# 1mishra/cbc

Hardware: AMD Instinct MI355X
Metric: Mbases/s encoded (bit-exact) on synthetic 150 bp SAM (higher is better)
Workload: dtype u32; 1 GPU; cfg2: synthetic 150 bp SAM, 10000000 reads per GPU vs a 248956422 bp uniform-ACGT contig, block-parallel encode; reads_rank0=10000000, blocks_rank0=2442, block_reads=4096, lds_bytes_per_block=15264, payload_bytes_rank0=20710203, parallelism=one GPU, no collective

## Files before the change

cbc_amd/csrc/cbc_encode_body.h:

```cpp
#ifndef CBC_ENCODE_BODY_H
#define CBC_ENCODE_BODY_H

#include <stdint.h>
#include <type_traits>
#include "../../include/cbc_gpu.h"
#include "cbc_plan.h"

#ifndef CBC_PRIO_CODER
#define CBC_PRIO_CODER 3
#define CBC_PRIO_MODEL 0
#endif
#define CBC_REC_PACK_AT 56u
#define CBC_AWORD     26u
#define CBC_M26       ((1u << 26) - 1u)
#define CBC_M25       ((1u << 25) - 1u)
#define CBC_RESCALE   (1u << 20)
#define CBC_NVARCTX   0xffffu
#define CBC_NOMEMO    0xffffffffu
#define CBC_BLOOM_LOG2 13u
#define CBC_ROLE_FUSED 0u
#define CBC_ROLE_MODEL 1u
#define CBC_ROLE_CODER 2u

#define CBC_LT_MATCH   0u
// ... 68 lines not shown
}

template <class W>
struct CbcWin {
    typedef typename W::V32 V32;
#ifndef CBC_WIN_SCALAR
    V32 w;
    CBC_MFN void clear() { w = W::splat(0u); }
    CBC_MFN void shift(uint32_t d)
    {
        if (d == 0u) return;
        if (d >= 256u) { clear(); return; }
        const V32 ln = W::lane();
        const V32 src = ln + (d >> 5);
        const V32 lo = W::lane_gather(w, src), hi = W::lane_gather(w, src + 1u);
        w = W::select(ln < 8u, W::funnel_shr(hi, lo, d & 31u), W::splat(0u));
    }
    CBC_MFN uint32_t first(uint32_t p, uint32_t rl)
    {
        uint32_t out = rl + 2u;
        if (p >= rl) return out;
        const V32 ln = W::lane();
        const uint32_t pw = p >> 5;
        const V32 a = W::select(ln == pw, w & (0xffffffffu << (p & 31u)), W::select(ln > pw, w, W::splat(0u)));
        const uint64_t hb = W::ballot(a != 0u);
        if (hb) {
            const uint32_t hl = W::ctz64(hb);
            const uint32_t pos = hl * 32u + W::ctz64((uint64_t)W::readlane(a, hl));
            if (pos < rl) out = pos - p;
        }
        return out;
    }
    CBC_MFN void set(uint32_t k)
    {
        if (k < 256u) w = w | W::select(W::lane() == (k >> 5), W::splat(1u << (k & 31u)), W::splat(0u));
    }
#else
    uint64_t w0, w1, w2, w3;
    CBC_MFN void clear() { w0 = w1 = w2 = w3 = 0; }
    CBC_MFN void shift(uint32_t d)
    {
        if (d == 0u) return;
        if (d >= 256u) { clear(); return; }
        uint32_t wsh = d >> 6, bsh = d & 63u;
        if (wsh == 1u) { w0 = w1; w1 = w2; w2 = w3; w3 = 0; }
        else if (wsh == 2u) { w0 = w2; w1 = w3; w2 = 0; w3 = 0; }
        else if (wsh == 3u) { w0 = w3; w1 = 0; w2 = 0; w3 = 0; }
        if (bsh) {
            uint32_t inv = 64u - bsh;
            w0 = (w0 >> bsh) | (w1 << inv);
            w1 = (w1 >> bsh) | (w2 << inv);
            w2 = (w2 >> bsh) | (w3 << inv);
            w3 = w3 >> bsh;
        }
    }
    CBC_MFN uint32_t first(uint32_t p, uint32_t rl)
    {
        uint32_t out = rl + 2u;
        if (p >= rl) return out;
        uint32_t pw = p >> 6; uint64_t pm = ~0ull << (p & 63u);
        uint64_t a0 = pw == 0u ? (w0 & pm) : 0ull;
        uint64_t a1 = pw == 1u ? (w1 & pm) : (pw < 1u ? w1 : 0ull);
        uint64_t a2 = pw == 2u ? (w2 & pm) : (pw < 2u ? w2 : 0ull);
        uint64_t a3 = pw == 3u ? (w3 & pm) : w3;
        uint32_t pos = 0xffffffffu;
        if (a0) pos = W::ctz64(a0);
        else if (a1) pos = 64u + W::ctz64(a1);
        else if (a2) pos = 128u + W::ctz64(a2);
        else if (a3) pos = 192u + W::ctz64(a3);
        if (pos < rl) out = pos - p;
        return out;
    }
    CBC_MFN void set(uint32_t k)
    {
        uint64_t bit = 1ull << (k & 63u); uint32_t kw = k >> 6;
        w0 |= (kw == 0u) ? bit : 0ull;
        w1 |= (kw == 1u) ? bit : 0ull;
        w2 |= (kw == 2u) ? bit : 0ull;
        w3 |= (kw == 3u) ? bit : 0ull;
    }
#endif
};

template <class W, bool GEN = false>
struct CbcEnc {
    typedef typename W::V32 V32;
    typedef typename W::Mask Mask;

    typedef typename W::Uv Uv;
    Uv l, rng;
    Uv lm1;
    Uv thr0;
    CBC_MFN void set_l_forms()
    {
        lm1 = W::uv_opaque(l - 1u);
        thr0 = ((l & (1u << 24)) | (1u << 25)) - l;
    }
    uint32_t scale3;
    uint32_t bitpos, flushed;
    uint32_t *ring;
    uint32_t *out32; uint32_t cap_words;
    uint32_t status, nsym, fail_read, cur_read;
    V32 q_lo, q_cnt, q_n; uint32_t q_len;
    uint32_t role, batch_i; uint32_t *batch, *ctl;
    V32 b_lo, b_hi, b_n, b_fl, b_fh; uint32_t b_len, b_pos, b_stop, b_flags, seen_last; uint64_t b_neq;
    V32 rec_a, rec_s; uint32_t rec_n;
#ifdef CBC_STAMP
    unsigned long long t_last, t_sum[16];
#endif

    V32 small;
    V32 fkey, fexc; uint32_t fcount;
    V32 hkey, hexc; uint32_t hc0, hc1, hc2, hc3, hn0, hn1, hn2, hn3;
    uint32_t *rlen_exc, *snps_exc, *indels_exc, *rname_key, *rname_exc, *pos_val, *pos_occ, *pos_pre, *pos_idx, *var_ev, *bloom, *p0ev;
    uint32_t *runs;
    uint32_t snps_n, indels_n;
    uint32_t rn_count, rn_cap;
    uint32_t *vtab;
    uint32_t *fsp_key, *fsp_exc; uint32_t fsp_count;
    uint32_t *pos_ov_val, *pos_ov_occ; uint32_t pos_lds_cap;
    uint32_t *palpha; uint32_t pa_n0, pa_n1, pa_n2, pa_n3;
    uint32_t pos_card, cap_pos;
    uint32_t nev, nev1, cap_var;
    V32 p0cnt; uint32_t p0over;
    uint32_t L0;

    uint32_t prevPos, prevM, prevChar, win_pos;
    CbcWin<W> win;

    CBC_MFN void fail(uint32_t st) { if (status == CBC_ST_OK) { status = st; fail_read = cur_read; } }

    CBC_MFN void place(const V32 &val, const V32 &len, const V32 &off, const Mask &m)
    {
        const V32 aligned = val << (W::splat(32u) - len);
        const V32 sh = off & 31u, w = (off >> 5) & (CBC_RING_WORDS - 1u);
        const Mask on = m & (len != 0u);
        W::lds_or(ring, w, aligned >> sh, on);
        W::lds_or(ring, (w + 1u) & (CBC_RING_WORDS - 1u), aligned << (W::splat(32u) - sh), on & (sh != 0u));
    }
    CBC_MFN void flush_full()
    {
        const V32 ln = W::lane();
        while ((bitpos >> 5) - flushed >= 64u) {
            const V32 idx = (ln + flushed) & (CBC_RING_WORDS - 1u);
            const V32 wv = W::load32(ring, idx, W::all(), 0u);
            if (flushed + 64u <= cap_words) W::store32(out32, ln + flushed, W::bswap_v(wv), W::all());
            else fail(CBC_ST_OUT_FULL);
            W::store32(ring, idx, W::splat(0u), W::all());
            flushed += 64u;
        }
    }
    CBC_MFN void put(uint32_t v, uint32_t n)
    {
        if (n == 0) return;
        place(W::splat(v), W::splat(n), W::splat(bitpos), W::lane() == 0u);
        bitpos += n;
        flush_full();
    }
    CBC_MFN void put_run(uint32_t bit, uint32_t n)
    {
        uint32_t pat = bit ? 0xffffffffu : 0u;
        while (n >= 32u) { put(pat, 32u); n -= 32u; }
        if (n) put(pat >> (32u - n), n);
    }
    CBC_MFN void pack(const V32 &rec_a, const V32 &rec_k3, uint32_t m)
    {
#ifdef CBC_ABLATE_PACK
        bitpos += m; return;
#endif
        const V32 ln = W::lane();
        const Mask in = ln < m;
        const V32 k1 = rec_a >> 26, bits = (rec_a & CBC_M26) >> ((W::splat(26u) - k1) & 31u);
        const Mask act = in & (k1 != 0u);
        const V32 k3 = W::select(in, rec_k3, W::splat(0u));
        const V32 s_in = W::scan_incl_add(k3), s_ex = s_in - k3;
        const V32 mark = W::select(act, s_ex + 1u, W::splat(0u));
        const V32 m_in = W::scan_incl_max(mark);
        const V32 m_ex = W::shift_up1(m_in, 0u);
        const V32 rec_s = W::select(m_ex == 0u, s_ex + scale3, s_ex - (m_ex - 1u));
        {
            const uint32_t total = W::readlane(s_in, 63u), last = W::readlane(m_in, 63u);
            scale3 = last ? total - (last - 1u) : scale3 + total;
        }
        const V32 len = W::select(act, k1 + rec_s, W::splat(0u));
#ifndef CBC_PACK_SERIAL_AT
#define CBC_PACK_SERIAL_AT 32u
#endif
        if (W::ballot(act & (len > CBC_PACK_SERIAL_AT))) {
            for (uint32_t k = 0; k < m; k++) {
                const uint32_t kk = W::readlane(k1, k), bb = W::readlane(bits, k), sc = W::readlane(rec_s, k);
                if (kk == 0u) continue;
                if (sc == 0u) put(bb, kk);
                else {
                    const uint32_t b0 = bb >> (kk - 1u);
                    put(b0, 1u); put_run(b0 ^ 1u, sc);
                    put(bb & ((1u << (kk - 1u)) - 1u), kk - 1u);
                }
            }
            return;
        }
        const V32 incl = W::scan_incl_add(len);
        const V32 km1 = (k1 - 1u) & 31u;
        const V32 b0 = bits >> km1;
        const V32 rest = bits & ((W::splat(1u) << km1) - 1u);
        const V32 run = W::select(b0 != 0u, W::splat(0u), (W::splat(1u) << rec_s) - 1u);
        const V32 val = (b0 << ((rec_s + km1) & 31u)) | (run << km1) | rest;
        place(val, len, incl - len + bitpos, act);
        bitpos += W::readlane(incl, 63u);
        flush_full();
    }

    CBC_MFN void encode(uint32_t lo, uint32_t cnt, uint32_t n)
    {
#ifdef CBC_EMU_TRACE
        cbc_emu_trace(cur_read, lo, cnt, n);
#endif
        V32 ln = W::lane();
        Mask here = ln == q_len;
        q_lo = W::select(here, W::splat(lo), q_lo);
        q_cnt = W::select(here, W::splat(cnt), q_cnt);
        q_n = W::select(here, W::splat(n), q_n);
        q_len++;
    }
#define CBC_FRAC(c, n) W::frac32(c, n)
#define CBC_BF_LAST  1u
#define CBC_BF_GROUP 2u
#define CBC_END_N    0xffffffffu
    CBC_MFN void drain() { if (role == CBC_ROLE_MODEL) publish(0u, 0ull); else drain_q(); }
    CBC_MFN void seg_end()
    {
        if (role != CBC_ROLE_MODEL) { drain_q(); return; }
        if (q_len >= 64u) publish(0u, 0ull);
        V32 ln = W::lane();
        Mask here = ln == q_len;
        q_lo = W::select(here, W::splat(0u), q_lo); q_cnt = W::select(here, W::splat(1u), q_cnt);
        q_n = W::select(here, W::splat(CBC_END_N), q_n);
        q_len++;
    }
    CBC_MFN void seg_end_fits()
    {
        W::expect_eq(q_len < 64u ? 1u : 0u, 1u, "seg_end_fits: queue full");
        V32 ln = W::lane();
        Mask here = ln == q_len;
        q_lo = W::select(here, W::splat(0u), q_lo); q_cnt = W::select(here, W::splat(1u), q_cnt);
        q_n = W::select(here, W::splat(CBC_END_N), q_n);
        q_len++;
    }
    CBC_MFN void publish(uint32_t flags, uint64_t neq)
    {
        V32 ln = W::lane();
        CBC_TSM(5);
        while (batch_i - W::ctl_load(ctl + 1) >= CBC_BATCH_SLOTS) W::nap();
        CBC_TSM(6);
        uint32_t *buf = batch + (batch_i & (CBC_BATCH_SLOTS - 1u)) * CBC_BATCH_WORDS;
        Mask m = ln < q_len;
        W::store32(buf, ln, q_lo, m); W::store32(buf + 64u, ln, q_cnt, m); W::store32(buf + 128u, ln, q_n, m);
        V32 hdr = W::select(ln == 0u, W::splat(q_len), W::select(ln == 1u, W::splat(flags),
                  W::select(ln == 2u, W::splat(status), W::select(ln == 3u, W::splat(status == CBC_ST_OK ? cur_read : fail_read),
                  W::select(ln == 4u, W::splat((uint32_t)neq), W::splat((uint32_t)(neq >> 32)))))));
        W::store32(buf + 192u, ln, hdr, ln < 6u);
        batch_i++;
        W::ctl_store(ctl, batch_i);
        q_len = 0;
    }
    CBC_MFN void step(uint32_t lo, uint32_t hi, uint32_t n, uint32_t flo, uint32_t fhi)
    {
        Uv rec, k3;
        code1(lo, hi, n, flo, fhi, rec, k3);
        W::set_lane_uv(rec_a, rec_n, rec);
        W::set_lane_uv(rec_s, rec_n, k3);
        nsym++;
        if (++rec_n >= CBC_REC_PACK_AT) { pack(rec_a, rec_s, rec_n); rec_n = 0; }
    }
    CBC_MFN void flush_recs() { if (rec_n) { pack(rec_a, rec_s, rec_n); rec_n = 0; } }
    CBC_MFN void room(uint32_t k) { if (rec_n + k >= 64u) flush_recs(); }
    template <class FLO, class FHI, class FN>
    CBC_MFN void step_fixed(FLO lo_of, FHI hi_of, FN n_of, uint32_t flo, uint32_t fhi)
    {
        Uv rec, k3;
        code1_lazy(flo, fhi, lo_of, hi_of, n_of, rec, k3);
#ifdef CBC_ABLATE_SETLANE
        rec_a ^= rec; rec_s ^= k3;
#else
        W::set_lane_uv(rec_a, rec_n, rec);
        W::set_lane_uv(rec_s, rec_n, k3);
#endif
        nsym++; rec_n++;
    }
    CBC_MFN void drain_q()
    {
        V32 ln = W::lane();
        uint32_t m = W::uni(q_len);
        const uint64_t bad = W::ballot((ln < m) & ((q_cnt == 0u) | (q_n == 0u)));
        if (bad) m = W::ctz64(bad);
        const V32 q_hi = q_lo + q_cnt;
        const V32 f_lo = CBC_FRAC(q_lo, q_n), f_hi = CBC_FRAC(q_hi, q_n);
        for (uint32_t k = 0; k < m; k++)
            step(W::readlane(q_lo, k), W::readlane(q_hi, k), W::readlane(q_n, k), W::readlane(f_lo, k), W::readlane(f_hi, k));
        if (bad) fail(CBC_ST_ASSERT);
        q_len = 0;
    }
    CBC_MFN void pull()
    {
        V32 ln = W::lane();
        CBC_TSM(9);
        while (W::ctl_load(ctl) == batch_i) W::nap();
        CBC_TSM(10);
        const uint32_t *buf = batch + (batch_i & (CBC_BATCH_SLOTS - 1u)) * CBC_BATCH_WORDS;
        V32 hdr = W::load32(buf + 192u, ln, ln < 6u, 0u);
        const uint32_t len = W::readlane(hdr, 0u);
        const uint32_t pst = W::readlane(hdr, 2u), prec = W::readlane(hdr, 3u);
        b_flags = W::readlane(hdr, 1u);
        b_neq = (uint64_t)W::readlane(hdr, 4u) | ((uint64_t)W::readlane(hdr, 5u) << 32);
        Mask m = ln < len;
        b_lo = W::load32(buf, ln, m, 0u); b_n = W::load32(buf + 128u, ln, m, 1u);
        const V32 cnt = W::load32(buf + 64u, ln, m, 1u);
        b_hi = b_lo + cnt;
        b_fl = CBC_FRAC(b_lo, b_n); b_fh = CBC_FRAC(b_hi, b_n);
        b_len = len > 64u ? 64u : len; b_pos = 0;
        const uint64_t bad = W::ballot(m & ((cnt == 0u) | (b_n == 0u)));
        b_stop = bad ? W::ctz64(bad) : 64u;
        batch_i++;
        W::ctl_store(ctl + 1, batch_i);
        if (b_flags & CBC_BF_LAST) seen_last = 1u;
        if (pst != CBC_ST_OK && status == CBC_ST_OK) { status = pst; fail_read = prec; }
    }
    CBC_MFN void seg_consume()
    {
        const V32 ln = W::lane();
        uint32_t done = 0u;
        while ((done | status) == 0u) {
            if (b_pos == b_len) {
                if (seen_last) fail(CBC_ST_ASSERT);
                else { pull(); if (b_flags & CBC_BF_GROUP) fail(CBC_ST_ASSERT); }
            } else {
                const uint64_t em = W::ballot((b_n == CBC_END_N) & (ln >= b_pos) & (ln < b_len));
                uint32_t kend = em ? W::ctz64(em) : b_len;
                const uint32_t bad = b_stop < kend ? 1u : 0u;
                if (bad) kend = b_stop;
                for (uint32_t k = b_pos; k < kend; k++) {
                    Uv rec, k3;
                    code1_lazy(W::readlane(b_fl, k), W::readlane(b_fh, k), [&]() -> uint32_t { return W::readlane(b_lo, k); },
                               [&]() -> uint32_t { return W::readlane(b_hi, k); }, [&]() -> uint32_t { return W::readlane(b_n, k); }, rec, k3);
                    W::set_lane_uv(rec_a, rec_n, rec);
                    W::set_lane_uv(rec_s, rec_n, k3);
                    nsym++;
                    if (++rec_n >= CBC_REC_PACK_AT) { pack(rec_a, rec_s, rec_n); rec_n = 0; }
                }
                if (bad) fail(CBC_ST_ASSERT);
                else if (em) { b_pos = kend + 1u; done = 1u; }
                else b_pos = kend;
            }
        }
    }
    CBC_MFN void consume_all()
    {
        while (!seen_last) {
            pull();
            if (status != CBC_ST_OK) continue;
            const uint32_t kend = b_stop < b_len ? b_stop : b_len;
            for (uint32_t k = 0; k < kend; k++) {
                Uv rec, k3;
                code1_lazy(W::readlane(b_fl, k), W::readlane(b_fh, k), [&]() -> uint32_t { return W::readlane(b_lo, k); },
                           [&]() -> uint32_t { return W::readlane(b_hi, k); }, [&]() -> uint32_t { return W::readlane(b_n, k); }, rec, k3);
                W::set_lane_uv(rec_a, rec_n, rec);
                W::set_lane_uv(rec_s, rec_n, k3);
                nsym++;
                if (++rec_n >= CBC_REC_PACK_AT) { pack(rec_a, rec_s, rec_n); rec_n = 0; }
            }
            if (b_stop < b_len) fail(CBC_ST_ASSERT);
        }
    }
    CBC_MFN void post_group(uint32_t g, uint64_t neq, uint32_t refused)
    {
        W::write_uni(ctl, 4u + 2u * (g & 1u), (uint32_t)neq);
        W::write_uni(ctl, 5u + 2u * (g & 1u), (uint32_t)(neq >> 32));
        if (refused) W::write_uni(ctl, 3u, 1u);
        W::ctl_store(ctl + 2, g + 1u);
    }
    CBC_MFN void abort_groups()
    {
        W::write_uni(ctl, 3u, 1u);
        W::ctl_store(ctl + 2, 0xffffffffu);
    }
    CBC_MFN bool wait_group(uint32_t g, uint64_t &neq)
    {
        CBC_TSM(5);
        while (W::ctl_load(ctl + 2) < g + 1u) W::nap();
        CBC_TSM(6);
        neq = (uint64_t)W::read_uni(ctl, 4u + 2u * (g & 1u)) | ((uint64_t)W::read_uni(ctl, 5u + 2u * (g & 1u)) << 32);
        return W::read_uni(ctl, 3u) == 0u;
    }
    CBC_MFN uint64_t pull_group()
    {
        if (status != CBC_ST_OK) return 0ull;
        if (b_pos != b_len || seen_last) { fail(CBC_ST_ASSERT); return 0ull; }
        pull();
        if (status == CBC_ST_OK && !(b_flags & CBC_BF_GROUP)) fail(CBC_ST_ASSERT);
        return b_neq;
    }
    CBC_MFN void pull_rest() { while (!seen_last) pull(); }
    CBC_MFN void code1(uint32_t lo, uint32_t hi, uint32_t n, uint32_t flo, uint32_t fhi, Uv &rec, Uv &k3)
    {
        code1_lazy(flo, fhi, [&]() { return lo; }, [&]() { return hi; }, [&]() { return n; }, rec, k3);
    }
    template <class FLO, class FHI, class FN>
    CBC_MFN void code1_lazy(uint32_t flo, uint32_t fhi, FLO lo_of, FHI hi_of, FN n_of, Uv &rec, Uv &k3)
    {
#ifdef CBC_ABLATE_CODER
        l ^= flo; rng ^= fhi; rec = W::uv(0u); k3 = rec; return;
#endif
        const Uv range = rng;
        Uv ql, qh, tl, th;
        W::mul64(range, flo, ql, tl); W::mul64(range, fhi, qh, th);
        if (W::uv_ge(tl | th, 0xfc000000u)) {
            const uint32_t lo = lo_of(), hi = hi_of(), n = n_of();
            ql += (range * lo - ql * n >= n) ? 1u : 0u;
            qh += (range * hi - qh * n >= n) ? 1u : 0u;
        }
#ifndef __HIP_DEVICE_COMPILE__
        W::expect_eq(W::uv_scalar(ql), (uint32_t)((uint64_t)W::uv_scalar(range) * lo_of() / n_of()), "scaled_div(cum)");
        W::expect_eq(W::uv_scalar(qh), (uint32_t)((uint64_t)W::uv_scalar(range) * hi_of() / n_of()), "scaled_div(cum + count)");
#endif
        code_tail(ql, qh, rec, k3);
    }
    CBC_MFN void code_tail(Uv ql, Uv qh, Uv &rec, Uv &k3)
    {
        const Uv u = lm1 + qh;
        l = l + ql;
        const Uv x = l ^ u;
        const Uv nya = ((~l | u) << 7) | 127u;
        const Uv k1 = W::clz_uv((x << 6) | 32u);
        rec = l | (k1 << 26);
        k3 = W::clz_uv(nya << k1);
        const Uv sh = k1 + k3;
        l = (l << sh) & CBC_M25;
        rng = (qh - ql) << sh;
        set_l_forms();
#ifndef __HIP_DEVICE_COMPILE__
        W::expect_eq(W::uv_scalar(l + rng - 1u), W::uv_scalar(((u << sh) & CBC_M25) | (1u << 25) | ((1u << sh) - 1u)), "range form of the upper bound");
#endif
    }
    template <class FHI, class FN>
    CBC_MFN void step_known0(FHI hi_of, FN n_of, uint32_t fhi)
    {
#ifdef CBC_ABLATE_CODER
        rng ^= fhi; nsym++; return;
#endif
        Uv qh, th;
        W::mul64(rng, fhi, qh, th);
        if (W::uv_ge(th, 0xfc000000u)) {
            const uint32_t hi = hi_of(), n = n_of();
            qh += (rng * hi - qh * n >= n) ? 1u : 0u;
        }
#ifndef __HIP_DEVICE_COMPILE__
        W::expect_eq(W::uv_scalar(qh), (uint32_t)((uint64_t)W::uv_scalar(rng) * hi_of() / n_of()), "scaled_div(count0)");
#endif
        nsym++;
        if (W::uv_gt(qh, thr0)) {
#ifndef __HIP_DEVICE_COMPILE__
            const uint32_t lf = W::uv_scalar(l), uf = lf + W::uv_scalar(qh) - 1u;
            W::expect_eq(((lf ^ uf) >> 25) & 1u, 1u, "step_known0: E1/E2 would shift");
            W::expect_eq((lf >> 24) & (~uf >> 24) & 1u, 0u, "step_known0: E3 would shift");
#endif
            rng = qh;
            return;
        }
        Uv rec, k3;
        code_tail(W::uv(0u), qh, rec, k3);
        W::set_lane_uv(rec_a, rec_n, rec);
        W::set_lane_uv(rec_s, rec_n, k3);
        rec_n++;
    }
    CBC_MFN uint32_t finish()
    {
        const uint32_t lf = W::uv_scalar(l);
        uint32_t msb = lf >> 25;
        put(msb, 1u); put_run(msb ^ 1u, scale3); scale3 = 0u;
        put(lf & CBC_M25, 25u);
        const uint32_t nbytes = (bitpos >> 3) + 1u;
        const uint32_t nw = (nbytes + 3u) >> 2;
        const V32 ln = W::lane();
        if (nw > cap_words) { fail(CBC_ST_OUT_FULL); return nbytes; }
        while (flushed < nw) {
            const V32 idx = (ln + flushed) & (CBC_RING_WORDS - 1u);
            const V32 wv = W::load32(ring, idx, W::all(), 0u);
            W::store32(out32, ln + flushed, W::bswap_v(wv), (ln + flushed) < nw);
            flushed += 64u;
        }
        return nbytes;
    }

    CBC_MFN void regsparse_code(V32 &key, V32 &exc, uint32_t base, uint32_t cap, uint32_t &count, uint32_t &n,
                               uint32_t card, uint32_t step, uint32_t x, uint32_t cap_status)
    {
        V32 ln = W::lane();
        Mask live = (ln >= base) & (ln < base + count);
        uint32_t lo = x + W::reduce_add(W::select(live & (key < x), exc, W::splat(0u)));
        uint64_t eq = W::ballot(live & (key == x));
        uint32_t idx = 0, cnt = 1u;
        if (eq) { idx = W::ctz64(eq); cnt = 1u + W::readlane(exc, idx); }
        if (x >= card) { fail(CBC_ST_ASSERT); return; }
        encode(lo, cnt, n);
        if (eq) exc = W::select(ln == idx, exc + step, exc);
        else {
            if (count >= cap) { fail(cap_status); return; }
            idx = base + count;
            key = W::select(ln == idx, W::splat(x), key);
            exc = W::select(ln == idx, W::splat(step), exc);
            count++;
        }
        n += step;
        if (n >= CBC_RESCALE) {
            live = (ln >= base) & (ln < base + count);
            exc = W::select(live, (exc + 1u) >> 1, exc);
            n = card + W::reduce_add(W::select(live, exc, W::splat(0u)));
        }
    }

    CBC_MFN void dense_lookup(const uint32_t *exc, uint32_t x, uint32_t &lo, uint32_t &cnt)
    {
        V32 ln = W::lane();
        if (x < 64u) {
            const V32 e = W::load32(exc, ln, ln <= x, 0u);
            cnt = 1u + W::readlane(e, x);
            if (x < 4u) { lo = x; for (uint32_t s = 0; s < x; s++) lo += W::readlane(e, s); }
            else lo = x + W::reduce_add(W::select(ln < x, e, W::splat(0u)));
            return;
        }
        V32 a = W::splat(0u);
        const uint32_t xb = W::uni(x);
        for (uint32_t b = 0; b < xb; b += 64u) { V32 i = ln + b; a = a + W::load32(exc, i, i < x, 0u); }
        lo = x + W::reduce_add(a);
        cnt = 1u + W::read_uni(exc, x);
    }
    CBC_MFN void dense_rescale(uint32_t *exc, uint32_t card, uint32_t &n)
    {
        V32 ln = W::lane();
        V32 a = W::splat(0u);
        const uint32_t cb = W::uni(card);
        for (uint32_t b = 0; b < cb; b += 64u) {
            V32 i = ln + b; Mask m = i < card;
            V32 e = (W::load32(exc, i, m, 0u) + 1u) >> 1;
            W::store32(exc, i, e, m);
            a = a + W::select(m, e, W::splat(0u));
        }
        n = card + W::reduce_add(a);
    }
    CBC_MFN void dense_code(uint32_t *exc, uint32_t card, uint32_t step, uint32_t x, uint32_t &n)
    {
        if (x >= card) { fail(CBC_ST_ASSERT); return; }
        uint32_t lo, cnt;
        dense_lookup(exc, x, lo, cnt);
        encode(lo, cnt, n);
// ... 899 lines not shown
        if (E.status == CBC_ST_OK) { gen_header(); E.seg_end(); }
        for (uint32_t c0 = 0; c0 < n_reads && E.status == CBC_ST_OK; c0 += 64u) {
            V32 r_pos, r_fl, r_seq, r_tok;
            const uint32_t cn = n_reads - c0 < 64u ? n_reads - c0 : 64u;
            E.cur_read = c0;
#ifndef CBC_MATCH_IN_MODEL
            if (E.q_len) E.publish(0u, 0ull);
            uint64_t neq;
            if (!E.wait_group(c0 >> 6, neq)) { E.fail(CBC_ST_ASSERT); break; }
            load_group(c0, r_pos, r_fl, r_seq, r_tok, false);
            CBC_TS(0);
#else
            if (!load_group(c0, r_pos, r_fl, r_seq, r_tok, true)) break;
            const uint64_t neq = match_group(cn, r_pos, r_fl, r_seq);
            CBC_TS(0);
            if (E.q_len) E.publish(0u, 0ull);
            E.publish(CBC_BF_GROUP, neq);
#endif
            if (c0 == 0u) { gen_rname(); E.seg_end(); }
            typename CbcEnc<W>::Prep P;
            E.prep_group(P, neq, r_tok, tokb, n_tok_blk);
            CBC_TS(14);
            uint64_t todo = neq;
            V32 nx_seq = W::splat(0u), nx_tok = W::splat(0u);
            uint32_t nx_j = 64u;
            auto prefetch = [&](uint32_t jn) {
                const uint32_t so = W::readlane(r_seq, jn), to = W::readlane(r_tok, jn), nrl = W::readlane(r_fl, jn) >> 16;
                V32 bo = ln * 4u;
                nx_seq = W::load32_bytes(seqb + so, bo, bo < nrl);
                nx_tok = W::load32(tokb + to, ln, (ln + to) < n_tok_blk, 0u);
                nx_j = jn;
            };
            auto prefetch_if_general = [&](uint64_t rest) {
                if (rest) { const uint32_t jn = W::ctz64(rest); if (!((P.ord >> jn) & 1ull)) prefetch(jn); }
            };
            typename CbcEnc<W>::Run R;
            R.pk = W::splat(0u); R.ca = R.pk; R.cb = R.pk; R.rm = 0ull; R.s = 0u; R.counted = 0u;
            while (todo && E.status == CBC_ST_OK) {
                const uint32_t j = W::ctz64(todo);
                if ((P.ord >> j) & 1ull) {
                    if (!E.run_pass(R, P, todo, r_pos, r_fl, r_seq, r_tok, tokb, seqb)) { P.ord &= ~R.rm; continue; }
                    todo &= ~R.rm;
                    prefetch_if_general(todo);
                    CBC_TS(2);
                    for (uint64_t rr = R.rm; rr && E.status == CBC_ST_OK; rr &= rr - 1ull) {
                        const uint32_t jr = W::ctz64(rr);
                        E.cur_read = c0 + jr;
                        E.run_record(R, W::readlane(P.hdr0, jr) >> 16, W::readlane(P.lo, jr), W::readlane(P.cnt, jr));
                        E.seg_end_fits();
                        CBC_TS(1);
                        if (E.q_len >= CBC_BATCH_MIN) E.drain();
                    }
                    continue;
                }
                if (nx_j != j) prefetch(j);
                todo &= todo - 1ull;
                E.cur_read = c0 + j;
                const V32 seqv = nx_seq, tokv = nx_tok;
                prefetch_if_general(todo);
                const typename CbcEnc<W>::PrepRec pr = { W::readlane(P.lo, j), W::readlane(P.cnt, j) };
                E.edits(W::readlane(r_pos, j), W::readlane(r_fl, j), W::readlane(r_tok, j), seqv, tokv, tokb, n_tok_blk, pr);
                E.seg_end_fits();
                CBC_TS(1);
                if (E.q_len >= CBC_BATCH_MIN) E.drain();
            }
        }
        if (E.status == CBC_ST_OK) { gen_sentinel(); E.seg_end(); }
#if defined(CBC_STAMP) && defined(__HIP_DEVICE_COMPILE__)
        if (E.cap_var >= 64u) for (int i = 0; i < 16; i++) {
            W::write_uni(E.var_ev + E.cap_var - 32u, 2 * i, (uint32_t)E.t_sum[i]); W::write_uni(E.var_ev + E.cap_var - 32u, 2 * i + 1, (uint32_t)(E.t_sum[i] >> 32)); }
#endif
        E.publish(CBC_BF_LAST, 0ull);
        return;
    }

    const bool fused = ROLE == CBC_ROLE_FUSED;
    if (!fused) W::prio(CBC_PRIO_CODER);
#ifndef CBC_MATCH_IN_MODEL
    uint64_t neq_ahead = 0;
    auto look_ahead = [&](uint32_t g0) {
        V32 a_pos, a_fl, a_seq, a_tok;
        const uint32_t an = n_reads - g0 < 64u ? n_reads - g0 : 64u;
        const uint32_t saved = E.cur_read;
        const bool okg = load_group(g0, a_pos, a_fl, a_seq, a_tok, true);
        neq_ahead = okg ? match_group(an, a_pos, a_fl, a_seq) : 0ull;
        E.post_group(g0 >> 6, neq_ahead, okg ? 0u : 1u);
        if (okg) E.cur_read = saved;
    };
    if (!fused && n_reads != 0u && E.status == CBC_ST_OK) look_ahead(0u);
#endif
    if (E.status == CBC_ST_OK) { if (fused) { gen_header(); E.seg_end(); } else E.seg_consume(); }
    for (uint32_t c0 = 0; c0 < n_reads && E.status == CBC_ST_OK; c0 += 64u) {
        V32 r_pos, r_fl, r_seq, r_tok;
        const uint32_t cn = n_reads - c0 < 64u ? n_reads - c0 : 64u;
        E.cur_read = c0;
        uint64_t neq;
        typename CbcEnc<W>::Prep P;
        typename CbcEnc<W>::Run R;
        R.pk = W::splat(0u); R.ca = R.pk; R.cb = R.pk; R.rm = 0ull; R.s = 0u; R.counted = 0u;
        if (fused) {
            if (!load_group(c0, r_pos, r_fl, r_seq, r_tok, true)) break;
            neq = match_group(cn, r_pos, r_fl, r_seq);
            E.prep_group(P, neq, r_tok, tokb, n_tok_blk);
        } else {
#ifndef CBC_MATCH_IN_MODEL
            neq = neq_ahead;
            if (c0 + 64u < n_reads) look_ahead(c0 + 64u);
            if (E.status != CBC_ST_OK) break;
#else
            neq = E.pull_group();
            if (E.status != CBC_ST_OK) break;
#endif
            load_group(c0, r_pos, r_fl, r_seq, r_tok, false);
        }
        typename CbcEnc<W>::Fixed F;
        E.fixed_group(F, c0, cn, r_pos, r_fl, neq);
        const V32 rdv = ln + c0;
        const V32 sr_hi = rdv * 10u - 9u, sr_n = rdv * 10u + 2u;
        const V32 sr_fh = CBC_FRAC(sr_hi, sr_n);
        const V32 t_hi = rdv * 10u + 1u, t_n = rdv * 10u + 255u;
        const V32 t_fh = CBC_FRAC(t_hi, t_n);
        const V32 rl_hi = F.rl_lo + F.rl_cnt;
        const V32 rl_fl = CBC_FRAC(F.rl_lo, t_n), rl_fh = CBC_FRAC(rl_hi, t_n);
        const V32 p_n = (F.p_card - 1u) * 10u + rdv * 10u + 1u, p_hi = F.p_lo + F.p_cnt;
        const V32 p_fl = CBC_FRAC(F.p_lo, p_n), p_fh = CBC_FRAC(p_hi, p_n);
        const V32 fl_n = rdv * 8u + 65536u, fl_hi = F.fl_lo + F.fl_cnt;
        const V32 fl_fl = CBC_FRAC(F.fl_lo, fl_n), fl_fh = CBC_FRAC(fl_hi, fl_n);
        const V32 m_hi = F.m_lo + F.m_cnt;
        const V32 m_fl = CBC_FRAC(F.m_lo, F.m_n), m_fh = CBC_FRAC(m_hi, F.m_n);

#ifndef CBC_ENC_NO_PEEL
#define CBC_ENC_FIRST(first, r) (decltype(first)::value)
#else
#define CBC_ENC_FIRST(first, r) ((r) == 0u)
#endif
#define CBC_LZ(expr) [&]() -> uint32_t { return (expr); }
        auto code_record = [&](uint32_t j, auto first, auto esc) {
            const uint32_t r = c0 + j;
            E.cur_read = r;
            E.room(8u);
            if (!CBC_ENC_FIRST(first, r)) E.step_known0(CBC_LZ(W::readlane(sr_hi, j)), CBC_LZ(10u * r + 2u), W::readlane(sr_fh, j));
            else {
                E.encode(1u, 1u, 2u); E.drain_q();
                if (fused) { gen_rname(); E.seg_end(); } else E.seg_consume();
            }
            {
                const uint32_t tn = 255u + 10u * r, tf = W::readlane(t_fh, j);
                E.step_fixed(CBC_LZ(W::readlane(F.rl_lo, j)), CBC_LZ(W::readlane(rl_hi, j)), CBC_LZ(tn), W::readlane(rl_fl, j), W::readlane(rl_fh, j));
                E.step_known0(CBC_LZ(W::readlane(t_hi, j)), CBC_LZ(tn), tf);
                E.step_known0(CBC_LZ(W::readlane(t_hi, j)), CBC_LZ(tn), tf);
                E.step_known0(CBC_LZ(W::readlane(t_hi, j)), CBC_LZ(tn), tf);
            }
            E.step_fixed(CBC_LZ(W::readlane(F.p_lo, j)), CBC_LZ(W::readlane(p_hi, j)), CBC_LZ(W::readlane(p_n, j)), W::readlane(p_fl, j), W::readlane(p_fh, j));
            if (decltype(esc)::value == 1 || (decltype(esc)::value == 2 && ((F.esc >> j) & 1ull))) {
                const uint32_t card = W::readlane(F.p_card, j);
                E.pos_alpha(W::read_uni(E.pos_val, card), card);
                E.drain_q();
            }
            E.step_fixed(CBC_LZ(W::readlane(F.fl_lo, j)), CBC_LZ(W::readlane(fl_hi, j)), CBC_LZ(65536u + 8u * r), W::readlane(fl_fl, j), W::readlane(fl_fh, j));
            E.step_fixed(CBC_LZ(W::readlane(F.m_lo, j)), CBC_LZ(W::readlane(m_hi, j)), CBC_LZ(W::readlane(F.m_n, j)), W::readlane(m_fl, j), W::readlane(m_fh, j));
            if ((neq >> j) & 1ull) {
                if (fused) {
                    if (((P.ord >> j) & 1ull) && !((R.rm >> j) & 1ull) &&
                        !E.run_pass(R, P, neq & (~0ull << j), r_pos, r_fl, r_seq, r_tok, tokb, seqb)) P.ord &= ~R.rm;
                    if ((P.ord >> j) & 1ull) E.run_record(R, W::readlane(P.hdr0, j) >> 16, W::readlane(P.lo, j), W::readlane(P.cnt, j));
                    else {
                        const uint32_t so = W::readlane(r_seq, j), to = W::readlane(r_tok, j), flw = W::readlane(r_fl, j);
                        const V32 bo = ln * 4u;
                        const V32 seqv = W::load32_bytes(seqb + so, bo, bo < (flw >> 16));
                        const V32 tokv = W::load32(tokb + to, ln, (ln + to) < n_tok_blk, 0u);
                        const typename CbcEnc<W>::PrepRec pr = { W::readlane(P.lo, j), W::readlane(P.cnt, j) };
                        E.edits(W::readlane(r_pos, j), flw, to, seqv, tokv, tokb, n_tok_blk, pr);
                    }
                    E.seg_end();
                } else E.seg_consume();
            }
        };
#undef CBC_LZ
        uint32_t jn = cn;
        if (F.bad) { const uint32_t fb = W::ctz64(F.bad); if (fb < cn) jn = fb; }
#ifndef CBC_ENC_NO_PEEL
        typedef std::integral_constant<int, 0> Plain; typedef std::integral_constant<int, 1> Esc; typedef std::integral_constant<int, 2> Look;
        uint32_t j = 0;
        if (c0 == 0u && jn != 0u) { code_record(0u, std::true_type(), Look()); j = 1u; }
        while (j < jn && E.status == CBC_ST_OK) {
            const uint64_t ahead = F.esc >> j;
            uint32_t run_end = ahead ? j + W::ctz64(ahead) : jn;
            if (run_end > jn) run_end = jn;
            for (; j < run_end && E.status == CBC_ST_OK; j++) code_record(j, std::false_type(), Plain());
            if (j < jn && E.status == CBC_ST_OK) { code_record(j, std::false_type(), Esc()); j++; }
        }
#else
        for (uint32_t j = 0; j < jn && E.status == CBC_ST_OK; j++) code_record(j, 0, std::integral_constant<int, 2>());
#endif
#undef CBC_ENC_FIRST
        if (jn < cn && E.status == CBC_ST_OK) { E.cur_read = c0 + jn; E.fail(W::readlane(F.st, jn)); }
    }
    uint32_t nbytes = 0;
    if (E.status == CBC_ST_OK) {
        E.cur_read = n_reads;
        if (n_reads) E.encode(10u * n_reads - 9u, 11u, 10u * n_reads + 2u);
        else E.encode(1u, 1u, 2u);
        E.drain_q();
        if (fused) { gen_sentinel(); E.seg_end(); } else E.seg_consume();
    }
    if (E.status == CBC_ST_OK) { E.flush_recs(); nbytes = E.finish(); }
    if (E.status != CBC_ST_OK) nbytes = 0;
#ifndef CBC_MATCH_IN_MODEL
#ifndef CBC_MATCH_NO_ABORT_FOR_TEST
    if (!fused && E.status != CBC_ST_OK) E.abort_groups();
#endif
#endif
    if (!fused) E.pull_rest();
#if defined(CBC_STAMP) && defined(__HIP_DEVICE_COMPILE__)
    if (payload_cap >= 128u) for (int i = 0; i < 16; i++) {
        W::write_uni(E.out32, 2 * i, (uint32_t)E.t_sum[i]); W::write_uni(E.out32, 2 * i + 1, (uint32_t)(E.t_sum[i] >> 32)); }
#endif
    V32 resv = W::select(ln == 0u, W::splat(nbytes), W::select(ln == 1u, W::splat(E.status),
               W::select(ln == 2u, W::splat(E.nsym), W::splat(E.fail_read))));
    W::store32((uint32_t *)(A.results + blk), ln, resv, ln < 4u);
}

#endif
```

cbc_amd/csrc/cbc_gpu.hip:

```cpp
#include <hip/hip_runtime.h>
#include <stdio.h>
#include <stdlib.h>
#include <string.h>
#include <stdint.h>
#include <new>
#include <time.h>
#include <dlfcn.h>
#include <rccl/rccl.h>

#include "../../include/cbc_gpu.h"
#include "cbc_wave_gpu.h"
#include "cbc_encode_body.h"
#include "cbc_decode_body.h"
#include "cbc_region_body.h"
#include "cbc_sam_body.h"
#include "cbc_depth_body.h"
#include "cbc_targets_body.h"
#include "cbc_cov_body.h"
#include "cbc_covx_body.h"
#include "cbc_quant_body.h"
#include "cbc_hist_body.h"
#include "cbc_stats_body.h"
#include "cbc_plan.h"
#include "cbc_stream_body.h"
#include "cbc_long_body.h"
#include "cbc_tokenise.h"

#define API extern "C" __attribute__((visibility("default")))
#define CBC_CTX_STREAM ((void *)(uintptr_t)1)

extern __shared__ uint32_t cbc_lds[];

static __device__ __forceinline__ void cbc_encode_block(const cbc_enc_args &A)
{
    uint32_t blk = blockIdx.x;
    if (blk >= A.n_blocks) return;
    const uint32_t wid = (uint32_t)__builtin_amdgcn_readfirstlane((int)(threadIdx.x >> 6));
    if (wid == 0u) cbc_encode_stream<WaveGPU, CBC_ROLE_MODEL>(A, blk, cbc_lds);
    else cbc_encode_stream<WaveGPU, CBC_ROLE_CODER>(A, blk, cbc_lds);
}

__global__ void __launch_bounds__(128) __attribute__((amdgpu_waves_per_eu(5)))
cbc_encode_blocks_kernel(cbc_enc_args A) { cbc_encode_block(A); }

__global__ void __launch_bounds__(128) __attribute__((amdgpu_waves_per_eu(6)))
cbc_encode_blocks_kernel_w6(cbc_enc_args A) { cbc_encode_block(A); }

__global__ void __launch_bounds__(64)
cbc_decode_blocks_kernel(cbc_dec_args A)
{
    uint32_t blk = blockIdx.x;
    if (blk >= A.n_blocks) return;
    cbc_decode_stream<WaveGPU>(A, blk, cbc_lds);
}

__global__ void __launch_bounds__(64)
cbc_decode_blocks_span_kernel(cbc_dec_args A, uint32_t smax)
{
    uint32_t blk = blockIdx.x;
    if (blk >= A.n_blocks) return;
    cbc_decode_stream<WaveGPU, true>(A, blk, cbc_lds, smax);
}

__global__ void __launch_bounds__(64)
cbc_region_count_kernel(cbc_region_args A) { if (blockIdx.x < A.n_blocks) cbc_region_count<WaveGPU>(A, blockIdx.x); }

#define CBC_REGION_WAVES 4u
__global__ void __launch_bounds__(64 * CBC_REGION_WAVES)
cbc_region_write_kernel(cbc_region_args A)
{
    if (blockIdx.x >= A.n_blocks) return;
    cbc_region_write<WaveGPU>(A, blockIdx.x, (uint32_t)__builtin_amdgcn_readfirstlane((int)(threadIdx.x >> 6)), CBC_REGION_WAVES);
}

__global__ void __launch_bounds__(64)
cbc_sam_count_kernel(cbc_sam_args A) { if (blockIdx.x < A.R.n_blocks) cbc_sam_count<WaveGPU>(A, blockIdx.x); }

#define CBC_SAM_WAVES 4u
__global__ void __launch_bounds__(64 * CBC_SAM_WAVES)
cbc_sam_write_kernel(cbc_sam_args A)
{
    if (blockIdx.x >= A.R.n_blocks) return;
    cbc_sam_write<WaveGPU>(A, blockIdx.x, (uint32_t)__builtin_amdgcn_readfirstlane((int)(threadIdx.x >> 6)), CBC_SAM_WAVES);
}

__global__ void __launch_bounds__(64)
cbc_depth_mark_kernel(cbc_depth_args A) { if (blockIdx.x < A.R.n_blocks) cbc_depth_mark<WaveGPU>(A, blockIdx.x); }
__global__ void __launch_bounds__(64)
cbc_depth_tile_kernel(cbc_depth_args A) { cbc_depth_tile<WaveGPU>(A, blockIdx.x); }
__global__ void __launch_bounds__(64)
cbc_depth_compact_kernel(cbc_depth_args A) { cbc_depth_compact<WaveGPU>(A, blockIdx.x); }
__global__ void __launch_bounds__(64)
cbc_depth_count_kernel(cbc_depth_args A) { if (blockIdx.x < A.n_ttiles) cbc_depth_count<WaveGPU>(A, blockIdx.x); }
__global__ void __launch_bounds__(64)
cbc_depth_write_kernel(cbc_depth_args A) { cbc_depth_write<WaveGPU>(A, blockIdx.x); }

__global__ void __launch_bounds__(64)
cbc_targets_count_kernel(cbc_targets_args A) { if (blockIdx.x < A.S.R.n_blocks) cbc_targets_count<WaveGPU>(A, blockIdx.x); }
__global__ void __launch_bounds__(64 * CBC_REGION_WAVES)
cbc_targets_write_kernel(cbc_targets_args A)
{
    if (blockIdx.x >= A.S.R.n_blocks) return;
    cbc_targets_write<WaveGPU>(A, blockIdx.x, (uint32_t)__builtin_amdgcn_readfirstlane((int)(threadIdx.x >> 6)), CBC_REGION_WAVES);
}
__global__ void __launch_bounds__(64)
cbc_targets_sam_count_kernel(cbc_targets_args A) { if (blockIdx.x < A.S.R.n_blocks) cbc_targets_sam_count<WaveGPU>(A, blockIdx.x); }
__global__ void __launch_bounds__(64 * CBC_SAM_WAVES)
cbc_targets_sam_write_kernel(cbc_targets_args A)
{
// ... 2453 lines not shown
```

cbc_amd/csrc/cbc_wave_gpu.h:

```cpp
#ifndef CBC_WAVE_GPU_H
#define CBC_WAVE_GPU_H

#include <hip/hip_runtime.h>
#include <stdint.h>

#define CBC_FN __device__ __forceinline__
#define CBC_MFN __device__ __forceinline__

struct WaveGPU {
    typedef uint32_t V32;
    typedef bool     Mask;

    static CBC_FN V32 lane() { return __builtin_amdgcn_mbcnt_hi(~0u, __builtin_amdgcn_mbcnt_lo(~0u, 0u)); }
    static CBC_FN V32 splat(uint32_t x) { return x; }
    static CBC_FN Mask all() { return true; }
    static CBC_FN void barrier() { __syncthreads(); }
    static CBC_FN V32 select(Mask m, V32 a, V32 b) { return m ? a : b; }
    static CBC_FN uint64_t ballot(Mask m) { return __ballot(m); }
    static CBC_FN uint32_t uni(uint32_t x) { return (uint32_t)__builtin_amdgcn_readfirstlane((int)x); }
    static CBC_FN uint32_t to_scalar(uint32_t x)
    {
        asm volatile("" : "+v"(x));
        return (uint32_t)__builtin_amdgcn_readfirstlane((int)x);
    }
    static CBC_FN uint32_t readlane(V32 v, uint32_t k) { return (uint32_t)__builtin_amdgcn_readlane((int)v, (int)uni(k)); }

    static CBC_FN uint32_t reduce_add(V32 v)
    {
        int x = (int)v;
        x += __builtin_amdgcn_update_dpp(0, x, 0x111, 0xf, 0xf, false);
        x += __builtin_amdgcn_update_dpp(0, x, 0x112, 0xf, 0xf, false);
        x += __builtin_amdgcn_update_dpp(0, x, 0x114, 0xf, 0xf, false);
        x += __builtin_amdgcn_update_dpp(0, x, 0x118, 0xf, 0xf, false);
        x += __builtin_amdgcn_update_dpp(0, x, 0x142, 0xa, 0xf, false);
        x += __builtin_amdgcn_update_dpp(0, x, 0x143, 0xc, 0xf, false);
        return (uint32_t)__builtin_amdgcn_readlane(x, 63);
    }

    static CBC_FN V32 scan_incl_add(V32 v)
    {
        int x = (int)v;
        x += __builtin_amdgcn_update_dpp(0, x, 0x111, 0xf, 0xf, false);
        x += __builtin_amdgcn_update_dpp(0, x, 0x112, 0xf, 0xf, false);
        x += __builtin_amdgcn_update_dpp(0, x, 0x114, 0xf, 0xf, false);
        x += __builtin_amdgcn_update_dpp(0, x, 0x118, 0xf, 0xf, false);
        x += __builtin_amdgcn_update_dpp(0, x, 0x142, 0xa, 0xf, false);
        x += __builtin_amdgcn_update_dpp(0, x, 0x143, 0xc, 0xf, false);
        return (uint32_t)x;
    }

    static CBC_FN V32 prefix_popc(uint64_t m)
    {
        return __builtin_amdgcn_mbcnt_hi((uint32_t)(m >> 32), __builtin_amdgcn_mbcnt_lo((uint32_t)m, 0u));
    }
    static CBC_FN V32 shift_up1(V32 v, uint32_t fill)
    {
        uint32_t l = lane();
        uint32_t t = (uint32_t)__builtin_amdgcn_ds_bpermute((int)((l - 1u) << 2), (int)v);
        return l == 0u ? fill : t;
    }
    static CBC_FN V32 lane_gather(V32 v, V32 idx) { return (uint32_t)__builtin_amdgcn_ds_bpermute((int)(idx << 2), (int)v); }
    static CBC_FN V32 funnel_shr(V32 hi, V32 lo, uint32_t sh) { return __builtin_amdgcn_alignbit(hi, lo, sh); }
    static CBC_FN V32 mulhi(V32 a, V32 b) { return __umulhi(a, b); }
    static CBC_FN Mask lane_bit(uint64_t m)
    {
        uint32_t l = lane();
        uint32_t w = l < 32u ? (uint32_t)m : (uint32_t)(m >> 32);
        return ((w >> (l & 31u)) & 1u) != 0u;
    }
    static CBC_FN V32 frac32(V32 c, V32 n)
    {
        double q = (double)c * 4294967296.0 / (double)(n ? n : 1u);
        return q >= 4294967295.0 ? 0xffffffffu : (uint32_t)q;
    }
    static CBC_FN void lds_add(uint32_t *p, V32 idx, V32 val, Mask m) { if (m) __hip_atomic_fetch_add(p + idx, val, __ATOMIC_RELAXED, __HIP_MEMORY_SCOPE_WORKGROUP); }
    static CBC_FN void lds_or(uint32_t *p, V32 idx, V32 val, Mask m) { if (m) __hip_atomic_fetch_or(p + idx, val, __ATOMIC_RELAXED, __HIP_MEMORY_SCOPE_WORKGROUP); }
    static CBC_FN void lds_zero(uint32_t *p, V32 idx, Mask m) { if (m) p[idx] = 0u; }
    static CBC_FN V32 lds_read(const uint32_t *p, V32 idx, Mask m) { return m ? p[idx] : 0u; }
    static CBC_FN void set_lane(V32 &v, uint32_t k, uint32_t val) { v = lane() == k ? val : v; }
    static CBC_FN V32 bswap_v(V32 x) { return __builtin_bswap32(x); }
    typedef uint32_t Uv;
    static CBC_FN Uv uv(uint32_t x) { uint32_t r; asm volatile("v_mov_b32 %0, %1" : "=v"(r) : "v"(x)); return r; }
    static CBC_FN Uv uv_opaque(Uv x) { asm volatile("" : "+v"(x)); return x; }
    static CBC_FN uint32_t uv_scalar(Uv x) { return (uint32_t)__builtin_amdgcn_readfirstlane((int)x); }
    static CBC_FN bool uv_gt(Uv x, Uv y) { return __builtin_amdgcn_uicmp(x, y, 34) != 0ull; }
    static CBC_FN bool uv_ge(Uv x, uint32_t c) { return __builtin_amdgcn_uicmp(x, c, 35) != 0ull; }
    static CBC_FN void mul64(Uv a, uint32_t b, Uv &hi, Uv &lo) { uint64_t p = (uint64_t)a * b; hi = (uint32_t)(p >> 32); lo = (uint32_t)p; }
    static CBC_FN Uv clz_uv(Uv x) { return (uint32_t)__builtin_clz(x); }
    static CBC_FN void set_lane_uv(V32 &v, uint32_t k, Uv val) { v = lane() == k ? val : v; }
#ifndef CBC_DEC_STATE_SCALAR
    static CBC_FN Uv dv(uint32_t x) { return uv(x); }
    static CBC_FN bool dv_ge(Uv x, Uv y) { return __builtin_amdgcn_uicmp(x, y, 35) != 0ull; }
    static CBC_FN bool dv_gt(Uv x, Uv y) { return __builtin_amdgcn_uicmp(x, y, 34) != 0ull; }
    static CBC_FN bool dv_nz(Uv x) { return __builtin_amdgcn_uicmp(x, 0u, 33) != 0ull; }
    static CBC_FN uint32_t dv_scalar(Uv x) { return (uint32_t)__builtin_amdgcn_readfirstlane((int)x); }
    static CBC_FN V32 dvv(Uv x) { return x; }
#else
    static CBC_FN Uv dv(uint32_t x) { return x; }
    static CBC_FN bool dv_ge(Uv x, Uv y) { return x >= y; }
    static CBC_FN bool dv_gt(Uv x, Uv y) { return x > y; }
    static CBC_FN bool dv_nz(Uv x) { return x != 0u; }
    static CBC_FN uint32_t dv_scalar(Uv x) { return x; }
    static CBC_FN V32 dvv(Uv x) { return x; }
#endif
    static CBC_FN uint32_t ctl_load(const uint32_t *p)
    {
        return uni(__hip_atomic_load(p, __ATOMIC_ACQUIRE, __HIP_MEMORY_SCOPE_WORKGROUP));
    }
    static CBC_FN void ctl_store(uint32_t *p, uint32_t v)
    {
        if (lane() == 0) __hip_atomic_store(p, v, __ATOMIC_RELEASE, __HIP_MEMORY_SCOPE_WORKGROUP);
    }
    static CBC_FN void nap() { __builtin_amdgcn_s_sleep(2); }
    static CBC_FN void prio(int p) { if (p == 0) __builtin_amdgcn_s_setprio(0); else if (p == 1) __builtin_amdgcn_s_setprio(1); else if (p == 2) __builtin_amdgcn_s_setprio(2); else __builtin_amdgcn_s_setprio(3); }
    static CBC_FN void expect_eq(uint32_t, uint32_t, const char *) {}

    static CBC_FN V32 scan_incl_max(V32 v)
    {
        uint32_t x = v;
#define CBC_DPP_MAX(ctrl, rmask) { uint32_t y_ = (uint32_t)__builtin_amdgcn_update_dpp(0, (int)x, ctrl, rmask, 0xf, false); x = x > y_ ? x : y_; }
        CBC_DPP_MAX(0x111, 0xf) CBC_DPP_MAX(0x112, 0xf) CBC_DPP_MAX(0x114, 0xf) CBC_DPP_MAX(0x118, 0xf)
        CBC_DPP_MAX(0x142, 0xa) CBC_DPP_MAX(0x143, 0xc)
#undef CBC_DPP_MAX
        return x;
    }
    static CBC_FN V32 load32(const uint32_t *p, V32 idx, Mask m, uint32_t other) { return m ? p[idx] : other; }
    static CBC_FN void store32(uint32_t *p, V32 idx, V32 val, Mask m) { if (m) p[idx] = val; }
    typedef uint32_t __attribute__((aligned(1))) u32_unaligned;
    static CBC_FN V32 load32_bytes(const uint8_t *p, V32 byteoff, Mask m)
    {
        return m ? *(const u32_unaligned *)(p + byteoff) : 0u;
    }
    static CBC_FN V32 load8(const uint8_t *p, V32 byteoff, Mask m) { return m ? (uint32_t)p[byteoff] : 0u; }
    static CBC_FN void store8(uint8_t *p, V32 byteoff, V32 val, Mask m) { if (m) p[byteoff] = (uint8_t)val; }
    static CBC_FN void store32_bytes(uint8_t *p, V32 byteoff, V32 val, Mask m) { if (m) *(u32_unaligned *)(p + byteoff) = val; }
    static CBC_FN void store_rec(uint4 *p, V32 idx, Mask m, V32 a, V32 b, V32 c, V32 d) { if (m) p[idx] = make_uint4(a, b, c, d); }
    static CBC_FN void load_rec(const uint4 *p, V32 idx, Mask m, V32 &a, V32 &b, V32 &c, V32 &d)
    {
        uint4 r = m ? p[idx] : make_uint4(0, 0, 0, 0);
        a = r.x; b = r.y; c = r.z; d = r.w;
    }
    static CBC_FN V32 load32_list(const uint32_t *p, V32 idx, Mask m, uint32_t other)
    {
        return m ? __hip_atomic_load(p + idx, __ATOMIC_RELAXED, __HIP_MEMORY_SCOPE_AGENT) : other;
    }
    static CBC_FN void store32_list(uint32_t *p, V32 idx, V32 val, Mask m)
    {
        if (m) __hip_atomic_store(p + idx, val, __ATOMIC_RELAXED, __HIP_MEMORY_SCOPE_AGENT);
    }
    static CBC_FN void list_add(uint32_t *p, V32 idx, V32 val, Mask m)
    {
        if (m) __hip_atomic_fetch_add(p + idx, val, __ATOMIC_RELAXED, __HIP_MEMORY_SCOPE_AGENT);
    }
    static CBC_FN void append_list(uint32_t *p, uint32_t idx, uint32_t val)
    {
        if (lane() == 0) __hip_atomic_store(p + idx, val, __ATOMIC_RELAXED, __HIP_MEMORY_SCOPE_AGENT);
    }
    static CBC_FN void list_fence() { __builtin_amdgcn_s_waitcnt(0x0f70);  }
    static CBC_FN uint32_t read_uni(const uint32_t *p, uint32_t idx) { return uni(p[idx]); }
    static CBC_FN uint32_t read_uni8(const uint8_t *p, uint32_t idx) { return uni((uint32_t)p[idx]); }
    static CBC_FN void write_uni(uint32_t *p, uint32_t idx, uint32_t val) { if (lane() == 0) p[idx] = val; }

    static CBC_FN void muldiv2(uint32_t range, uint32_t lo, uint32_t hi, uint32_t n, float inv,
                               uint32_t &ql, uint32_t &qh)
    {
        uint32_t c = lane() == 0u ? hi : lo;
        uint32_t plo = range * c, phi = __umulhi(range, c);
        float pf = (float)((phi << 16) | (plo >> 16)) * 65536.0f;
        uint32_t q0 = (uint32_t)(pf * inv);
        int32_t r0 = (int32_t)(plo - q0 * n);
        int32_t q1 = (int32_t)__builtin_floorf((float)r0 * inv);
        int32_t r1 = r0 - q1 * (int32_t)n;
// ... 39 lines not shown
```

Baseline: 226,200 Mbases/s.

## Add quiet fixed-step coder path and shared-mask lane insertion helpers

Result: faster. 234,700 Mbases/s, median of 6 (+3.8%).

```diff
diff --git a/cbc_amd/csrc/cbc_encode_body.h b/cbc_amd/csrc/cbc_encode_body.h
--- a/cbc_amd/csrc/cbc_encode_body.h
+++ b/cbc_amd/csrc/cbc_encode_body.h
@@ -174,6 +174,9 @@
 #endif
 };
 
+template <class W, class = void> struct CbcHasLaneN : std::false_type {};
+template <class W> struct CbcHasLaneN<W, std::void_t<decltype(&W::set_lane2_uv), decltype(&W::set_lane3)>> : std::true_type {};
+
 template <class W, bool GEN = false>
 struct CbcEnc {
     typedef typename W::V32 V32;
@@ -307,12 +310,24 @@
 #ifdef CBC_EMU_TRACE
         cbc_emu_trace(cur_read, lo, cnt, n);
 #endif
-        V32 ln = W::lane();
-        Mask here = ln == q_len;
-        q_lo = W::select(here, W::splat(lo), q_lo);
-        q_cnt = W::select(here, W::splat(cnt), q_cnt);
-        q_n = W::select(here, W::splat(n), q_n);
+        q_put(lo, cnt, n);
+    }
+    CBC_MFN void q_put(uint32_t lo, uint32_t cnt, uint32_t n)
+    {
+        if constexpr (!GEN && CbcHasLaneN<W>::value) W::set_lane3(q_lo, q_cnt, q_n, q_len, lo, cnt, n);
+        else {
+            V32 ln = W::lane();
+            Mask here = ln == q_len;
+            q_lo = W::select(here, W::splat(lo), q_lo);
+            q_cnt = W::select(here, W::splat(cnt), q_cnt);
+            q_n = W::select(here, W::splat(n), q_n);
+        }
         q_len++;
+    }
+    CBC_MFN void rec_put(Uv rec, Uv k3)
+    {
+        if constexpr (!GEN && CbcHasLaneN<W>::value) W::set_lane2_uv(rec_a, rec_s, rec_n, rec, k3);
+        else { W::set_lane_uv(rec_a, rec_n, rec); W::set_lane_uv(rec_s, rec_n, k3); }
     }
 #define CBC_FRAC(c, n) W::frac32(c, n)
 #define CBC_BF_LAST  1u
@@ -323,20 +338,12 @@
     {
         if (role != CBC_ROLE_MODEL) { drain_q(); return; }
         if (q_len >= 64u) publish(0u, 0ull);
-        V32 ln = W::lane();
-        Mask here = ln == q_len;
-        q_lo = W::select(here, W::splat(0u), q_lo); q_cnt = W::select(here, W::splat(1u), q_cnt);
-        q_n = W::select(here, W::splat(CBC_END_N), q_n);
-        q_len++;
+        q_put(0u, 1u, CBC_END_N);
     }
     CBC_MFN void seg_end_fits()
     {
         W::expect_eq(q_len < 64u ? 1u : 0u, 1u, "seg_end_fits: queue full");
-        V32 ln = W::lane();
-        Mask here = ln == q_len;
-        q_lo = W::select(here, W::splat(0u), q_lo); q_cnt = W::select(here, W::splat(1u), q_cnt);
-        q_n = W::select(here, W::splat(CBC_END_N), q_n);
-        q_len++;
+        q_put(0u, 1u, CBC_END_N);
     }
     CBC_MFN void publish(uint32_t flags, uint64_t neq)
     {
@@ -359,8 +366,7 @@
     {
         Uv rec, k3;
         code1(lo, hi, n, flo, fhi, rec, k3);
-        W::set_lane_uv(rec_a, rec_n, rec);
-        W::set_lane_uv(rec_s, rec_n, k3);
+        rec_put(rec, k3);
         nsym++;
         if (++rec_n >= CBC_REC_PACK_AT) { pack(rec_a, rec_s, rec_n); rec_n = 0; }
     }
@@ -374,9 +380,43 @@
 #ifdef CBC_ABLATE_SETLANE
         rec_a ^= rec; rec_s ^= k3;
 #else
-        W::set_lane_uv(rec_a, rec_n, rec);
-        W::set_lane_uv(rec_s, rec_n, k3);
-#endif
+        rec_put(rec, k3);
+#endif
+        nsym++; rec_n++;
+    }
+    template <class FLO, class FHI, class FN>
+    CBC_MFN void step_fixed_quiet(FLO lo_of, FHI hi_of, FN n_of, uint32_t flo, uint32_t fhi)
+    {
+#ifdef CBC_ABLATE_CODER
+        step_fixed(lo_of, hi_of, n_of, flo, fhi); return;
+#endif
+        Uv ql, qh, tl, th;
+        W::mul64(rng, flo, ql, tl); W::mul64(rng, fhi, qh, th);
+        if (W::uv_ge(tl | th, 0xfc000000u)) {
+            const uint32_t lo = lo_of(), hi = hi_of(), n = n_of();
+            ql += (rng * lo - ql * n >= n) ? 1u : 0u;
+            qh += (rng * hi - qh * n >= n) ? 1u : 0u;
+        }
+#ifndef __HIP_DEVICE_COMPILE__
+        W::expect_eq(W::uv_scalar(ql), (uint32_t)((uint64_t)W::uv_scalar(rng) * lo_of() / n_of()), "scaled_div(cum), quiet step");
+        W::expect_eq(W::uv_scalar(qh), (uint32_t)((uint64_t)W::uv_scalar(rng) * hi_of() / n_of()), "scaled_div(cum + count), quiet step");
+#endif
+        const Uv l1 = l + ql, u = lm1 + qh;
+        const Uv still = (l1 ^ u) & ~((l1 & ~u) << 1);
+        if (W::uv_ge(still & (1u << 25), 1u)) {
+#ifndef __HIP_DEVICE_COMPILE__
+            const uint32_t lf = W::uv_scalar(l1), uf = W::uv_scalar(u);
+            W::expect_eq(W::clz32((((lf ^ uf) & CBC_M26) << 6) | 32u), 0u, "step_fixed_quiet: E1/E2 would shift");
+            W::expect_eq(W::clz32(((((~lf | uf) << 7) | 127u))), 0u, "step_fixed_quiet: E3 would shift");
+#endif
+            l = l1; rng = qh - ql;
+            set_l_forms();
+            nsym++;
+            return;
+        }
+        Uv rec, k3;
+        code_tail(ql, qh, rec, k3);
+        rec_put(rec, k3);
         nsym++; rec_n++;
     }
     CBC_MFN void drain_q()
@@ -434,8 +474,7 @@
                     Uv rec, k3;
                     code1_lazy(W::readlane(b_fl, k), W::readlane(b_fh, k), [&]() -> uint32_t { return W::readlane(b_lo, k); },
                                [&]() -> uint32_t { return W::readlane(b_hi, k); }, [&]() -> uint32_t { return W::readlane(b_n, k); }, rec, k3);
-                    W::set_lane_uv(rec_a, rec_n, rec);
-                    W::set_lane_uv(rec_s, rec_n, k3);
+                    rec_put(rec, k3);
                     nsym++;
                     if (++rec_n >= CBC_REC_PACK_AT) { pack(rec_a, rec_s, rec_n); rec_n = 0; }
                 }
@@ -455,8 +494,7 @@
                 Uv rec, k3;
                 code1_lazy(W::readlane(b_fl, k), W::readlane(b_fh, k), [&]() -> uint32_t { return W::readlane(b_lo, k); },
                            [&]() -> uint32_t { return W::readlane(b_hi, k); }, [&]() -> uint32_t { return W::readlane(b_n, k); }, rec, k3);
-                W::set_lane_uv(rec_a, rec_n, rec);
-                W::set_lane_uv(rec_s, rec_n, k3);
+                rec_put(rec, k3);
                 nsym++;
                 if (++rec_n >= CBC_REC_PACK_AT) { pack(rec_a, rec_s, rec_n); rec_n = 0; }
             }
@@ -560,8 +598,7 @@
         }
         Uv rec, k3;
         code_tail(W::uv(0u), qh, rec, k3);
-        W::set_lane_uv(rec_a, rec_n, rec);
-        W::set_lane_uv(rec_s, rec_n, k3);
+        rec_put(rec, k3);
         rec_n++;
     }
     CBC_MFN uint32_t finish()
@@ -1627,9 +1664,11 @@
         V32 a_pos, a_fl, a_seq, a_tok;
         const uint32_t an = n_reads - g0 < 64u ? n_reads - g0 : 64u;
         const uint32_t saved = E.cur_read;
+        CBC_TS(9);
         const bool okg = load_group(g0, a_pos, a_fl, a_seq, a_tok, true);
         neq_ahead = okg ? match_group(an, a_pos, a_fl, a_seq) : 0ull;
         E.post_group(g0 >> 6, neq_ahead, okg ? 0u : 1u);
+        CBC_TS(15);
         if (okg) E.cur_read = saved;
     };
     if (!fused && n_reads != 0u && E.status == CBC_ST_OK) look_ahead(0u);
@@ -1691,7 +1730,7 @@
             }
             {
                 const uint32_t tn = 255u + 10u * r, tf = W::readlane(t_fh, j);
-                E.step_fixed(CBC_LZ(W::readlane(F.rl_lo, j)), CBC_LZ(W::readlane(rl_hi, j)), CBC_LZ(tn), W::readlane(rl_fl, j), W::readlane(rl_fh, j));
+                E.step_fixed_quiet(CBC_LZ(W::readlane(F.rl_lo, j)), CBC_LZ(W::readlane(rl_hi, j)), CBC_LZ(tn), W::readlane(rl_fl, j), W::readlane(rl_fh, j));
                 E.step_known0(CBC_LZ(W::readlane(t_hi, j)), CBC_LZ(tn), tf);
                 E.step_known0(CBC_LZ(W::readlane(t_hi, j)), CBC_LZ(tn), tf);
                 E.step_known0(CBC_LZ(W::readlane(t_hi, j)), CBC_LZ(tn), tf);
diff --git a/cbc_amd/csrc/cbc_gpu.hip b/cbc_amd/csrc/cbc_gpu.hip
--- a/cbc_amd/csrc/cbc_gpu.hip
+++ b/cbc_amd/csrc/cbc_gpu.hip
@@ -25,6 +25,8 @@
 #include "cbc_stream_body.h"
 #include "cbc_long_body.h"
 #include "cbc_tokenise.h"
+
+static_assert(CbcHasLaneN<WaveGPU>::value, "WaveGPU must supply set_lane2_uv and set_lane3");
 
 #define API extern "C" __attribute__((visibility("default")))
 #define CBC_CTX_STREAM ((void *)(uintptr_t)1)
diff --git a/cbc_amd/csrc/cbc_wave_gpu.h b/cbc_amd/csrc/cbc_wave_gpu.h
--- a/cbc_amd/csrc/cbc_wave_gpu.h
+++ b/cbc_amd/csrc/cbc_wave_gpu.h
@@ -88,6 +88,17 @@
     static CBC_FN void mul64(Uv a, uint32_t b, Uv &hi, Uv &lo) { uint64_t p = (uint64_t)a * b; hi = (uint32_t)(p >> 32); lo = (uint32_t)p; }
     static CBC_FN Uv clz_uv(Uv x) { return (uint32_t)__builtin_clz(x); }
     static CBC_FN void set_lane_uv(V32 &v, uint32_t k, Uv val) { v = lane() == k ? val : v; }
+    static CBC_FN void cnd_e64(V32 &v, V32 val, uint64_t m) { asm("v_cndmask_b32_e64 %0, %0, %1, %2" : "+v"(v) : "v"(val), "s"(m)); }
+    static CBC_FN void set_lane2_uv(V32 &a, V32 &b, uint32_t k, Uv va, Uv vb)
+    {
+        const uint64_t m = __builtin_amdgcn_uicmp(lane(), k, 32);
+        cnd_e64(a, va, m); cnd_e64(b, vb, m);
+    }
+    static CBC_FN void set_lane3(V32 &a, V32 &b, V32 &c, uint32_t k, uint32_t va, uint32_t vb, uint32_t vc)
+    {
+        const uint64_t m = __builtin_amdgcn_uicmp(lane(), k, 32);
+        cnd_e64(a, va, m); cnd_e64(b, vb, m); cnd_e64(c, vc, m);
+    }
 #ifndef CBC_DEC_STATE_SCALAR
     static CBC_FN Uv dv(uint32_t x) { return uv(x); }
     static CBC_FN bool dv_ge(Uv x, Uv y) { return __builtin_amdgcn_uicmp(x, y, 35) != 0ull; }
```
